# jiahuei/COMIC-Compact-Image-Captioning-with-Attention

Hardware: AMD Instinct MI355X
Metric: images/sec (decoder-mode XE training, COMIC-256, InceptionV3 frozen) (higher is better)
Workload: dtype bf16

## Files before the change

### comic-compact-image-captioning-with-attention_amd/_lib.py

```python
import ctypes as C
import os

_HERE = os.path.dirname(os.path.abspath(__file__))
LIB_PATH = os.environ.get('COMIC_HIP_LIB') or os.path.join(_HERE, 'lib', 'libcomic_hip.so')

c_void_p, c_int, c_int32, c_int64, c_float, c_double, c_char_p, c_uint64 = (
    C.c_void_p, C.c_int, C.c_int32, C.c_int64, C.c_float, C.c_double, C.c_char_p, C.c_uint64)


class CnnOp(C.Structure):
    _fields_ = [(n, c_int32) for n in (
        'kind', 'src', 'dst', 'src_coff', 'dst_coff', 'H', 'W', 'Cin', 'Cout', 'KH', 'KW', 'SH', 'SW',
        'PT', 'PL', 'Ho', 'Wo', 'weight', 'relu', 'out_f32', 'src_f32', 'lane', 'tile', 'group', 'flags', 'min_lds')]


class ImageDesc(C.Structure):
    _fields_ = [('offset', C.c_int64), ('in_h', c_int32), ('in_w', c_int32), ('flip', c_int32), ('oy', c_int32),
                ('ox', c_int32), ('sy', C.c_float), ('sx', C.c_float)]


class ConvWeight(C.Structure):
    _fields_ = [('w', c_void_p), ('scale', c_void_p), ('shift', c_void_p), ('w_frag', c_void_p)]


# ... 69 lines not shown


class BeamSampling(C.Structure):
    _fields_ = [('temperature', c_float), ('seed_dev', c_void_p)]


class BeamTruncation(C.Structure):
    _fields_ = [('top_k', c_int32), ('top_p', c_float)]


class GemmProb(C.Structure):
    _fields_ = [(n, c_void_p) for n in ('A', 'B', 'C', 'bias', 'mask')] + [(n, c_int32) for n in (
        'M', 'N', 'K', 'lda', 'ldb', 'ldc', 'ld_mask')] + [(n, c_float) for n in ('alpha', 'beta', 'keep')] + [
        ('type', c_int32), ('ones_a', c_int32)]


class ConvGrad(C.Structure):
    _fields_ = [('w_master', c_void_p), ('dw', c_void_p), ('dbeta', c_void_p), ('w_bwd', c_void_p),
                ('bwd_tile', c_int32), ('reserved', c_int32)]


P = c_void_p
_SIGS = {
    'comic_last_error': (c_char_p, []),
    'comic_abi_version': (c_int, []),
    'comic_device_count': (c_int, []),
    'comic_pack_conv_weights': (c_int, [P, P, c_int, c_int, c_int, c_int, c_int, P]),
    'comic_fold_bn': (c_int, [P, P, P, c_float, P, P, c_int, P]),
    'comic_cnn_forward': (c_int, [P, c_int, P, P, P, c_int, c_int, P]),
    'comic_cnn_group_args_bytes': (C.c_long, [P, c_int]),
    'comic_cnn_build_group_args': (c_int, [P, c_int, P, P, P, c_int, P]),
    'comic_cnn_forward_grouped': (c_int, [P, c_int, P, P, P, c_int, c_int, P, P]),
    'comic_clip_by_norm': (c_int, [P, P, P, c_int, c_float, c_float, c_float, P, P, P]),
    'comic_cnn_backward_scratch_bytes': (c_int64, [P, c_int, c_int, c_int, c_int]),
    'comic_cnn_backward': (c_int, [P, c_int, P, P, P, P, P, c_int, c_int, c_int, P, c_int64, P, P]),
    'comic_cnn_backward_sched': (c_int, [P, c_int, P, c_int, P, P, P, P, P, P, c_int, c_int, c_int, P, c_int64, P, P, P]),
    'comic_cnn_pack_bwd_filters': (c_int, [P, c_int, P, c_int, P]),
    'comic_cnn_pack_x3_weights': (c_int, [P, P, P, P, P, c_int, P]),
    'comic_cnn_refresh_weights': (c_int, [P, P, c_int64, P, P, P, P, c_int64, P]),
    'comic_cnn_refresh_weights_dtype': (c_int, [P, P, c_int64, P, P, P, P, c_int64, c_int, P]),
    'comic_cnn_pack_frag_weights': (c_int, [P, P, P, c_int, c_int64, P]),
    'comic_crc32c': (C.c_uint32, [P, C.c_size_t, C.c_uint32]),
    'comic_conv2d_bn_relu': (c_int, [P, P, c_int, P, c_int, P, c_int, c_int, P]),
    'comic_gemm_f32': (c_int, [P, P, P, P, c_int, c_int, c_int, c_int, c_int, c_int, c_int, c_int, c_float,
                               c_float, P]),
    'comic_gemm_f32_split3': (c_int, [P, P, P, P, c_int, c_int, c_int, c_int, c_int, c_int, c_int, c_int, c_float,
                                      c_float, P, c_int64, P]),
    'comic_gemm_f32_splitk': (c_int, [P, P, P, P, c_int, c_int, c_int, c_int, c_int, c_int, c_int, c_int, c_float,
                                      c_float, P, c_int64, P]),
    'comic_gemm_group_workspace': (c_int64, [P, c_int]),
    'comic_gemm_group': (c_int, [P, c_int, P, c_int64, P]),
    'comic_gemm_group_form': (c_int, [P, c_int, P, c_int64, c_int, P]),
    'comic_gemm_group_resident': (c_int, [c_int]),
    'comic_embed_fwd': (c_int, [P, P, P, c_int, c_int, c_int, P]),
    'comic_embed_bwd': (c_int, [P, P, P, c_int, c_int, c_int, P]),
    'comic_dropout_apply': (c_int, [P, P, c_float, P, c_int64, P]),
    'comic_dropout_mask': (c_int, [P, c_int64, c_float, c_uint64, c_uint64, P]),
    'comic_dropout_mask_dev': (c_int, [P, c_int64, c_float, P, c_uint64, P]),
    'comic_dropout_masks4_dev': (c_int, [P, P, P, P, P]),
    'comic_image_preprocess': (c_int, [P, P, c_int, P, c_int, c_int, c_int, P]),
    'comic_jpeg_pixels': (c_int, [P, P, c_int, c_int, c_int, c_int, P, P, P]),
    'comic_jpeg_preprocess': (c_int, [P, P, c_int, c_int, P, P, P, P, c_int, c_int, c_int, P]),
    'comic_jpeg_preprocess_packed': (c_int, [P, P, c_int, c_int, P, P, P, P, c_int, c_int, c_int, P]),
    'comic_weighted_sum_tb': (c_int, [P, P, c_int, c_int, P, P]),
    'comic_lstm_gates_fwd': (c_int, [P, P, P, P, P, P, P, P, c_float, P, c_int, P, P, c_int, c_int, P]),
    'comic_lstm_gates_bwd': (c_int, [P, P, P, P, P, c_float, P, c_int, P, P, P, c_int, c_int, P]),
    'comic_attn_step_fwd': (c_int, [P, P, P, P, P, P, P, P, P, c_float, P, P, P, P]),
    'comic_attn_step_bwd': (c_int, [P, P, P, P, P, P, P, P, P, P, c_float, P, P, P, P, P, P, P]),
    'comic_xent_fwd_bwd': (c_int, [P, P, P, P, P, P, P, P, c_int, c_int, c_int, P]),
    'comic_argmax_rows': (c_int, [P, P, c_int, c_int, P]),
    'comic_beam_step': (c_int, [P, P, P, P, P, P, P, c_int, c_int, c_int, c_int, P]),
    'comic_gather_rows': (c_int, [P, P, P, c_int, c_int, c_int, P]),
    'comic_gather_tree': (c_int, [P, P, P, P, c_int, c_int, c_int, c_int, P]),
    'comic_adam_tf': (c_int, [P, P, P, P, c_int64, c_float, c_float, c_float, c_float, c_float, c_float, P]),
    'comic_adam_tf_gated': (c_int, [P, P, P, P, c_int64, c_float, c_float, c_float, c_float, c_float, c_float, P, P]),
    'comic_momentum_tf_gated': (c_int, [P, P, P, c_int64, c_float, c_float, c_float, c_float, P, P]),
    'comic_debug_occupy_cus': (c_int, [c_int, c_int, P]),
    'comic_colsum': (c_int, [P, P, c_int, c_int, c_float, P]),
    'comic_ln_tanh_fwd': (c_int, [P, P, P, P, P, c_int, c_int, c_float, P]),
    'comic_ln_tanh_bwd_rows': (c_int, [P, P, P, P, P, c_int, c_int, P]),
    'comic_momentum_tf': (c_int, [P, P, P, c_int64, c_float, c_float, c_float, c_float, P]),
    'comic_axpy': (c_int, [P, P, c_float, c_int64, P]),
    'comic_decoder_train_workspace': (c_int64, [P, c_int, c_int]),
    'comic_decoder_train_path': (c_int, []),
    'comic_decoder_greedy_path': (c_int, []),
    'comic_decoder_beam_path': (c_int, []),
    'comic_beam_step_dense_workspace': (c_int64, [c_int, c_int, c_int, c_int]),
    'comic_beam_step_dense': (c_int, [c_void_p] * 9 + [c_int] * 5 + [c_void_p, c_int64, c_void_p]),
    'comic_gemm_f32_stream_workspace': (c_int64, [c_int, c_int, c_int]),
    'comic_gemm_f32_stream': (c_int, [c_void_p, c_void_p, c_void_p, c_void_p, c_int, c_int, c_int, c_void_p, c_int64, c_void_p]),
    'comic_decoder_infer_workspace': (c_int64, [P, c_int, c_int]),
    'comic_decoder_train_step': (c_int, [P, P, P, P, P, P, P, P, P, P, c_int, c_int, c_int, P, P, P, P, P, P, P,
                                         P, P, P, P, P, c_int64, P]),
    'comic_decoder_score_workspace': (c_int64, [P, c_int, c_int]),
    'comic_decoder_score': (c_int, [P, P, P, P, P, P, P, P, c_int, c_int, c_int, P, P, P, P, c_int64, P]),
    'comic_decoder_score_path': (c_int, []),
    'comic_decoder_greedy': (c_int, [P, P, P, P, c_int, c_int, P, P, P, P, P, c_int64, P]),
    'comic_decoder_sample': (c_int, [P, P, P, P, c_int, c_int, P, P, P, P, P, P, c_int64, P]),
    'comic_decoder_beam': (c_int, [P, P, P, P, c_int, c_int, c_int, P, P, P, P, P, P, P, P, c_int64, P]),
    'comic_beam_step_ensemble_workspace': (c_int64, [c_int, c_int, c_int, c_int]),
    'comic_beam_step_ensemble': (c_int, [P, P, c_int, P, P, P, P, P, P, c_int, c_int, c_int, c_int, c_float, P, c_int64, P]),
    'comic_beam_step_ensemble_path': (c_int, []),
    'comic_decoder_beam_ensemble_workspace': (c_int64, [P, c_int, c_int, c_int]),
    'comic_decoder_beam_ensemble': (c_int, [P, P, P, P, P, c_int, c_int, c_int, c_int, P, P, P, P, P, P, P, P, c_int64, P]),
    'comic_beam_bans': (c_int, [P, P, P, P, P, P, c_int, c_int, c_int, c_int, c_int, c_int, P, P]),
    'comic_beam_step_constrained': (c_int, [P, P, c_int, P, P, P, P, P, P, c_int, c_int, c_int, c_int, c_float, P, c_int, P,
# ... 166 lines not shown
```

### comic-compact-image-captioning-with-attention_amd/csrc/decoder_exec.hip

```cpp
#include <atomic>
#include <stdlib.h>

#include <algorithm>
#include <string.h>

#include "common.h"
#include "decoder_math.h"
#include "decoder_persist.h"
#include "exec_entries.h"
#include "gemm_group.h"
#include "lstm_prep.h"
#include "lstm_stream_dev.h"

int comic_gemm_f32_ws(const float* A, const float* B, float* C, const float* bias, int M, int N, int K, int lda,
                      int ldb, int ldc, int trans_a, int trans_b, float alpha, float beta, void* ws, int64_t ws_bytes,
                      hipStream_t st);
int comic_embed_bwd_set(const int32_t* ids, const float* dout, float* dtable, int rows, int E, int V, hipStream_t st);
int comic_gemm_bf16x3_impl(const float* A, const float* B, float* C, const float* bias, int M, int N, int K, int lda,
                           int ldb, int ldc, int trans_a, int trans_b, float alpha, float beta, void* ws,
                           int64_t ws_bytes, hipStream_t st);
bool comic_score_stream_supported(int D, int V);
int64_t comic_score_logits_ws_bytes(int D, int V, long rows, int stream);
float* comic_score_logits_buffer(void* ws);
int comic_score_logits(const float* y, const float* W_o, const float* b_o, const int32_t* targets_bt, const float* wmask_bt,
// ... 407 lines not shown
  finished[i] = first ? 0 : 1;
  lengths[i] = 0;
}

__global__ void pad_rows_kernel(const float* __restrict__ in, float* __restrict__ out, int cols, int ld, long n) {
  const long i = (long)blockIdx.x * blockDim.x + threadIdx.x;
  if (i >= n) return;
  const long r = i / ld;
  const int c = (int)(i - r * ld);
  out[i] = c < cols ? in[r * cols + c] : 0.f;
}

inline int fill(float* p, float v, long n, hipStream_t st) {
  if (n <= 0) return 0;
  hipLaunchKernelGGL(fill_kernel, dim3((unsigned)cdiv64(n, 256)), dim3(256), 0, st, p, v, n);
  COMIC_LAUNCH_CHECK("fill");
  return 0;
}
constexpr int64_t kSplitKBytes = 32ll << 20;

inline int gemm(const float* A, const float* B, float* C, const float* bias, int M, int N, int K, int lda, int ldb,
                int ldc, int ta, int tb, float beta, hipStream_t st) {
  return comic_gemm_f32_ws(A, B, C, bias, M, N, K, lda, ldb, ldc, ta, tb, 1.0f, beta, g_splitk_ws,
                           g_splitk_ws ? kSplitKBytes : 0, st);
}

inline int gemm_big(const float* A, const float* B, float* C, const float* bias, int M, int N, int K, int lda, int ldb,
                    int ldc, int ta, int tb, float beta, hipStream_t st) {
  const bool on = !(g_dec_flags & COMIC_DEC_EXACT_GEMM);
  if (!on || (long)M * N < 64 * 256 || K < 64)
    return gemm(A, B, C, bias, M, N, K, lda, ldb, ldc, ta, tb, beta, st);
  return comic_gemm_bf16x3_impl(A, B, C, bias, M, N, K, lda, ldb, ldc, ta, tb, 1.0f, beta, g_splitk_ws,
                                g_splitk_ws ? kSplitKBytes : 0, st);
}

constexpr int kGroupTickets = 4096;
struct GemmGroupRun {
  ComicGemmGroup g{};
  ComicGemmProb* add(int type, const float* A, const float* B, float* C, int M, int N, int K, int lda, int ldb, int ldc) {
    if (g.n >= kGemmGroupMax) return nullptr;
    ComicGemmProb& p = g.p[g.n++];
    p = ComicGemmProb{};
    p.type = type; p.A = A; p.B = B; p.C = C; p.M = M; p.N = N; p.K = K; p.lda = lda; p.ldb = ldb; p.ldc = ldc;
    p.alpha = 1.f; p.beta = 0.f; p.keep = 1.f;
    return &p;
  }
  ComicGemmProb* add_colsum(const float* B, float* C, int N, int K, int ldb) {
    ComicGemmProb* p = add(COMIC_GG_TN, nullptr, B, C, 1, N, K, 1, ldb, N);
    if (p) p->ones_a = 1;
    return p;
  }
  int run(void* slab, int64_t slab_cap, unsigned* tickets, hipStream_t st) {
    if (g.n == 0) return 0;
    int target = kGemmGroupTargetItems;
    for (;;) {
      int64_t need = 0;
      int nt = 0;
      const int wg = comic_gemm_group_plan(g, target, &need, &nt);
      if (wg < 0) return 2;
      if (need <= slab_cap && nt <= kGroupTickets - 8) {
        g.slab = (float*)slab;
        g.tickets = tickets;
        return comic_gemm_group_launch(g, wg, st);
      }
      COMIC_REQUIRE(target > 1, "gemm_group: split-K scratch too small");
      target = target / 2;
    }
  }
};

int check_desc(const comic_decoder_desc* d) {
  COMIC_REQUIRE(d, "decoder: null descriptor");
  COMIC_REQUIRE(d->D > 0 && d->E > 0 && d->A > 0 && d->V > 1 && d->C > 0 && d->Cg > 0 && d->H > 0 && d->M > 0,
                "decoder: bad dimensions");
  const int cv = d->fm_projection == 0 ? d->C : d->D;
  COMIC_REQUIRE(d->Cv == cv, "decoder: Cv must be %d for fm_projection %d", cv, d->fm_projection);
  const int a = (d->fm_projection == 0 && !d->context_layer) ? d->C : d->D;
  COMIC_REQUIRE(d->A == a, "decoder: attention size A must be %d", a);
  COMIC_REQUIRE(d->cell >= COMIC_CELL_LSTM && d->cell <= COMIC_CELL_GRU, "decoder: unknown cell %d", d->cell);
  return 0;
}
int check_cell_params(const comic_decoder_desc* d, const comic_decoder_params* p) {
  COMIC_REQUIRE(p && p->K, "decoder: null cell kernel");
  if (d->cell == COMIC_CELL_LSTM) COMIC_REQUIRE(p->b, "decoder: LSTM needs its bias");
  if (d->cell == COMIC_CELL_LN_LSTM) COMIC_REQUIRE(p->cell_ln, "decoder: LN_LSTM needs cell_ln");
  if (d->cell == COMIC_CELL_GRU) COMIC_REQUIRE(p->b && p->K_c && p->b_c, "decoder: GRU needs b, K_c, b_c");
  return 0;
}

comic_attn_desc attn_desc(const comic_decoder_desc* d, int rows) {
  comic_attn_desc a;
  a.B = rows; a.M = d->M; a.D = d->D; a.H = d->H; a.Cv = d->Cv;
  a.method = d->method; a.prob = d->prob; a.tied = d->fm_projection == 2;
  return a;
}

int memory_projections(const comic_decoder_desc* d, const comic_decoder_params* p, const float* fm, int rows,
                       float* keys, float* values_buf, const float** values, hipStream_t st) {
  RC(gemm_big(fm, p->W_m, keys, nullptr, rows * d->M, d->D, d->C, d->C, d->D, d->D, 0, 0, 0.f, st));
  if (d->fm_projection == 2) {
    *values = keys;
  } else if (d->fm_projection == 1) {
    RC(gemm_big(fm, p->W_v, values_buf, nullptr, rows * d->M, d->D, d->C, d->C, d->D, d->D, 0, 0, 0.f, st));
    *values = values_buf;
  } else {
    *values = fm;
  }
  return 0;
}

struct InitBufs {
  float *x, *xh, *g, *gates, *c_new;
  float *lnx = nullptr, *lnr = nullptr;
};

int rnn_init_fwd(const comic_decoder_desc* d, const comic_decoder_params* p, const float* im_embed, int rows,
                 const float* mask_init, InitBufs& ib, float* c0, float* h0, hipStream_t st) {
  const int D = d->D, EA = d->E + d->A;
  if (d->init_method == 1) {
    RC(gemm(im_embed, p->W_init, h0, nullptr, rows, D, d->Cg, d->Cg, D, D, 0, 0, 0.f, st));
// ... 1655 lines not shown
```

### comic-compact-image-captioning-with-attention_amd/csrc/gemm_group.h

```cpp
#pragma once
#include "common.h"

constexpr int kGemmGroupMax = 20;
enum { COMIC_GG_TN = 0, COMIC_GG_NN = 1, COMIC_GG_NT = 2 };

struct ComicGemmProb {
  const float* A;
  const float* B;
  float* C;
  const float* bias;
  const float* mask;
  int M, N, K, lda, ldb, ldc, ld_mask;
  float alpha, beta;
  float keep;
  int type;
  int ones_a;
  int tiles_m, tiles_n, S, k_per_slice, wg_begin;
  int slab_tile0;
  int ticket0;
};

struct ComicGemmGroup {
  ComicGemmProb p[kGemmGroupMax];
  int n;
  float* slab;
  unsigned* tickets;
  int xcd_chunk;
};

int comic_gemm_group_plan(ComicGemmGroup& g, int target_items, int64_t* slab_bytes, int* n_tickets);
constexpr int kGemmGroupTargetItems = 640;
int comic_gemm_group_launch(const ComicGemmGroup& g, int n_wg, hipStream_t st, int form = 0);
```

### comic-compact-image-captioning-with-attention_amd/csrc/gemm_group.hip

```cpp
#include <algorithm>

#include "gemm_group.h"
#include "gemm_x3_dev.h"

namespace {

constexpr int GB = 128;
constexpr int kGemmGroupSlots = 512;
constexpr int kItemOverhead = 6;
constexpr int kSc1 = 16;
typedef __attribute__((ext_vector_type(4))) unsigned gg_u32x4_t;

__device__ __forceinline__ __amdgpu_buffer_rsrc_t gg_rsrc(const void* p, long bytes) {
  return __builtin_amdgcn_make_buffer_rsrc((void*)p, 0, (int)bytes, 0x00020000);
}
__device__ __forceinline__ float4 gg_load16_sc1(__amdgpu_buffer_rsrc_t r, unsigned off) {
  const gg_u32x4_t v = __builtin_amdgcn_raw_buffer_load_b128(r, (int)off, 0, kSc1);
  return make_float4(__uint_as_float(v.x), __uint_as_float(v.y), __uint_as_float(v.z), __uint_as_float(v.w));
}
__device__ __forceinline__ void gg_store16_sc1(__amdgpu_buffer_rsrc_t r, unsigned off, float4 v) {
  const gg_u32x4_t u = {__float_as_uint(v.x), __float_as_uint(v.y), __float_as_uint(v.z), __float_as_uint(v.w)};
  __builtin_amdgcn_raw_buffer_store_b128(u, r, (int)off, 0, kSc1);
}

constexpr int kGroupLds = 4 * (X3Tile<GB, true>::BYTES + X3Tile<GB, true>::BYTES);
static_assert(X3Tile<GB, true>::BYTES >= X3Tile<GB, false>::BYTES, "LDS of the k-contiguous form bounds the others");
constexpr int kGroupLdsPc = 2 * 2 * (X3TilePc<GB, false>::BYTES + X3TilePc<GB, false>::BYTES);
static_assert(X3TilePc<GB, false>::BYTES >= X3TilePc<GB, true>::BYTES, "LDS of the row-contiguous form bounds the others");

__device__ __forceinline__ void gg_emit(const ComicGemmProb& p, int m, int n, float4 a) {
  if (m >= p.M || n >= p.N) return;
  const int nv = min(4, p.N - n);
  float v[4] = {a.x * p.alpha, a.y * p.alpha, a.z * p.alpha, a.w * p.alpha};
  float* cp = p.C + (size_t)m * p.ldc + n;
#pragma unroll
  for (int q = 0; q < 4; ++q) {
    if (q >= nv) break;
    if (p.bias) v[q] += p.bias[n + q];
    if (p.mask) v[q] = (v[q] / p.keep) * p.mask[(size_t)m * p.ld_mask + n + q];
    if (p.beta != 0.f) v[q] += p.beta * cp[q];
  }
  if (nv == 4 && (p.ldc % 4 == 0) && (((uintptr_t)p.C & 15) == 0)) {
    *(float4*)cp = make_float4(v[0], v[1], v[2], v[3]);
  } else {
#pragma unroll
    for (int q = 0; q < 4; ++q)
      if (q < nv) cp[q] = v[q];
  }
}

template <int FORM>
__global__ __launch_bounds__(FORM == 1 ? 256 : 512)
#if defined(__HIP_DEVICE_COMPILE__)
__attribute__((amdgpu_waves_per_eu(FORM == 3 ? 4 : 1, FORM == 3 ? 4 : 2)))
#endif
void gemm_group_x3_kernel(ComicGemmGroup g) {
  constexpr bool PC = FORM != 1;
  constexpr int NT = PC ? 512 : 256;
  constexpr int LDS = PC ? kGroupLdsPc : kGroupLds;
  extern __shared__ __attribute__((aligned(16))) unsigned char smem[];
  int bid = blockIdx.x;
  if (g.xcd_chunk > 0 && bid < g.xcd_chunk * 8) bid = (bid & 7) * g.xcd_chunk + (bid >> 3);
  volatile unsigned* s_last = (volatile unsigned*)(smem + LDS - 16);
  int pi = 0;
#pragma unroll 1
  for (int i = 1; i < g.n; ++i)
    if (bid >= g.p[i].wg_begin) pi = i;
  const ComicGemmProb& p = g.p[pi];
  const int local = bid - p.wg_begin;
  const int S = p.S, ntiles = p.tiles_m * p.tiles_n;
  const int slice = local / ntiles, tl = local - slice * ntiles;
  constexpr int PW = 8;
  const int panel = tl / (p.tiles_m * PW), rem = tl - panel * p.tiles_m * PW;
  const int pw = min(PW, p.tiles_n - panel * PW);
  const int mt = rem / pw, nt = panel * PW + rem % pw;
  const int tile = mt * p.tiles_n + nt;
  const int m0 = mt * GB, n0 = nt * GB;
  const int kbeg = S > 1 ? slice * p.k_per_slice : 0;
  const int kend = S > 1 ? min(p.K, kbeg + p.k_per_slice) : p.K;
  const int tid = threadIdx.x, lane = tid & 63, wave = tid >> 6;
  const int wm = wave >> 1, wn = wave & 1;

  const long tile_id = (long)p.ticket0 + tile;
  const __amdgpu_buffer_rsrc_t sr = gg_rsrc(g.slab + ((long)p.slab_tile0 + (long)tile * S) * (GB * GB), (long)S * GB * GB * 4);
  const unsigned sbase = (unsigned)slice * (GB * GB * 4);
  if (p.ones_a) {
    constexpr int KG = 8;
    float4* red = (float4*)smem;
    const int cg = tid & 31, kg = tid >> 5, n = n0 + 4 * cg;
    const bool vec = (p.ldb % 4 == 0) && (((uintptr_t)p.B & 15) == 0);
    float4 sm = make_float4(0.f, 0.f, 0.f, 0.f);
    if (n < p.N && kg < KG)
      for (int k = kbeg + kg; k < kend; k += KG) {
        const float4 v = load4(p.B + (size_t)k * p.ldb + n, p.N - n, vec);
        sm.x += v.x; sm.y += v.y; sm.z += v.z; sm.w += v.w;
      }
    if (kg < KG) red[kg * 32 + cg] = sm;
    __syncthreads();
    if (tid < 32) {
      float4 tot = red[cg];
#pragma unroll
      for (int k = 1; k < KG; ++k) {
        const float4 v = red[k * 32 + cg];
        tot.x += v.x; tot.y += v.y; tot.z += v.z; tot.w += v.w;
      }
      if (S == 1) gg_emit(p, 0, n, tot);
      else gg_store16_sc1(sr, sbase + (unsigned)cg * 16u, tot);
    }
    if (S == 1) return;
  } else {
    f32x4_t acc[4][4];
    if constexpr (PC) {
      constexpr int DEPTH = FORM == 3 ? 2 : 4;
      if (p.type == COMIC_GG_TN) x3_mainloop_pc<false, false, DEPTH>(p.A, p.B, p.M, p.N, p.lda, p.ldb, m0, n0, kbeg, kend, smem, acc);
      else if (p.type == COMIC_GG_NN) x3_mainloop_pc<true, false, DEPTH>(p.A, p.B, p.M, p.N, p.lda, p.ldb, m0, n0, kbeg, kend, smem, acc);
      else x3_mainloop_pc<true, true, DEPTH>(p.A, p.B, p.M, p.N, p.lda, p.ldb, m0, n0, kbeg, kend, smem, acc);
    } else {
      if (p.type == COMIC_GG_TN)
        x3_mainloop<GB, false, false, GB>(p.A, p.B, p.M, p.N, p.lda, p.ldb, m0, n0, kbeg, kend, smem, acc);
      else if (p.type == COMIC_GG_NN)
        x3_mainloop<GB, true, false, GB>(p.A, p.B, p.M, p.N, p.lda, p.ldb, m0, n0, kbeg, kend, smem, acc);
      else
        x3_mainloop<GB, true, true, GB>(p.A, p.B, p.M, p.N, p.lda, p.ldb, m0, n0, kbeg, kend, smem, acc);
    }
    const bool owner = wave < 4;
    if (S == 1) {
      if (owner)
#pragma unroll
      for (int i = 0; i < 4; ++i)
#pragma unroll
        for (int j = 0; j < 4; ++j)
          gg_emit(p, m0 + wm * 64 + j * 16 + (lane & 15), n0 + wn * 64 + i * 16 + (lane >> 4) * 4,
                  make_float4(acc[i][j][0], acc[i][j][1], acc[i][j][2], acc[i][j][3]));
      return;
    }
    if (owner)
#pragma unroll
    for (int i = 0; i < 4; ++i)
#pragma unroll
      for (int j = 0; j < 4; ++j) {
        const int ml = wm * 64 + j * 16 + (lane & 15), nl = wn * 64 + i * 16 + (lane >> 4) * 4;
        gg_store16_sc1(sr, sbase + (unsigned)(ml * GB + nl) * 4u, make_float4(acc[i][j][0], acc[i][j][1], acc[i][j][2], acc[i][j][3]));
      }
  }
  asm volatile("s_waitcnt vmcnt(0)" ::: "memory");
  __syncthreads();
  if (tid == 0) {
    const unsigned t = __hip_atomic_fetch_add(g.tickets + tile_id, 1u, __ATOMIC_RELAXED, __HIP_MEMORY_SCOPE_AGENT);
    *s_last = (t == (unsigned)(S - 1)) ? 1u : 0u;
    if (t == (unsigned)(S - 1)) __hip_atomic_store(g.tickets + tile_id, 0u, __ATOMIC_RELAXED, __HIP_MEMORY_SCOPE_AGENT);
  }
  __syncthreads();
  if (!*s_last) return;
  const int n_chunks = p.ones_a ? 1 : (GB * GB / 4) / NT;
#pragma unroll 1
  for (int c = 0; c < n_chunks; c += 4) {
    float4 sum[4];
#pragma unroll
    for (int u = 0; u < 4; ++u) sum[u] = make_float4(0.f, 0.f, 0.f, 0.f);
#pragma unroll 1
    for (int s = 0; s < S; ++s) {
      float4 v[4];
#pragma unroll
      for (int u = 0; u < 4; ++u) v[u] = gg_load16_sc1(sr, (unsigned)s * (GB * GB * 4) + (unsigned)(tid + NT * (c + u)) * 16u);
#pragma unroll
      for (int u = 0; u < 4; ++u) {
        sum[u].x += v[u].x; sum[u].y += v[u].y; sum[u].z += v[u].z; sum[u].w += v[u].w;
      }
    }
#pragma unroll
    for (int u = 0; u < 4; ++u) {
      const int idx4 = tid + NT * (c + u);
      if (!p.ones_a || idx4 < GB / 4) gg_emit(p, m0 + idx4 / (GB / 4), n0 + (idx4 % (GB / 4)) * 4, sum[u]);
    }
  }
}


}

int comic_gemm_group_plan(ComicGemmGroup& g, int target_items, int64_t* slab_bytes, int* n_tickets) {
  COMIC_REQUIRE(g.n > 0 && g.n <= kGemmGroupMax, "gemm_group: %d problems", g.n);
  long cost = 0;
  for (int i = 0; i < g.n; ++i) {
    ComicGemmProb& p = g.p[i];
    COMIC_REQUIRE(p.M > 0 && p.N > 0 && p.K > 0 && p.B && p.C && (p.A || p.ones_a), "gemm_group: bad problem %d", i);
    COMIC_REQUIRE(p.type >= COMIC_GG_TN && p.type <= COMIC_GG_NT, "gemm_group: bad type of problem %d", i);
    COMIC_REQUIRE(!p.ones_a || (p.type == COMIC_GG_TN && p.M == 1), "gemm_group: ones_a needs type TN and M = 1 (problem %d)", i);
    COMIC_REQUIRE(p.ldc >= p.N && (!p.mask || p.ld_mask >= p.N), "gemm_group: leading dimension of problem %d", i);
    if (!p.ones_a) COMIC_REQUIRE(p.lda >= (p.type == COMIC_GG_TN ? p.M : p.K), "gemm_group: lda of problem %d", i);
    COMIC_REQUIRE(p.ldb >= (p.type == COMIC_GG_NT ? p.K : p.N), "gemm_group: ldb of problem %d", i);
    p.tiles_m = cdiv(p.M, GB);
    p.tiles_n = cdiv(p.N, GB);
    cost += (long)cdiv(p.M, GB) * p.tiles_n * cdiv(p.K, 32);
  }
  auto split_of = [](int kt, long klen) { return (int)std::min<long>(16, std::max<long>(1, (kt + klen / 2) / klen)); };
  long klen = std::max<long>(8, cost / std::max(1, target_items));
  {
    long best = -1, best_klen = klen, kt_max = 8;
    for (int i = 0; i < g.n; ++i) kt_max = std::max<long>(kt_max, cdiv(g.p[i].K, 32));
    for (long kl = klen; kl <= kt_max; ++kl) {
      long items = 0, longest = 0;
      for (int i = 0; i < g.n; ++i) {
        const ComicGemmProb& p = g.p[i];
        const int kt = cdiv(p.K, 32), S = split_of(kt, kl);
        items += (long)p.tiles_m * p.tiles_n * S;
        if (!p.ones_a) longest = std::max<long>(longest, cdiv(kt, S));
      }
      const long est = cdiv64(items, kGemmGroupSlots) * (longest + kItemOverhead);
      if (best < 0 || est < best) {
        best = est;
        best_klen = kl;
      }
    }
    klen = best_klen;
  }
  int wg = 0, tickets = 0, slab_tiles = 0;
  for (int i = 0; i < g.n; ++i) {
    ComicGemmProb& p = g.p[i];
    const int nt = cdiv(p.M, GB) * p.tiles_n, kt = cdiv(p.K, 32);
    int S = split_of(kt, klen);
    p.k_per_slice = cdiv(kt, S) * 32;
    S = cdiv(p.K, p.k_per_slice);
    p.S = S;
    p.wg_begin = wg;
    p.slab_tile0 = slab_tiles;
    p.ticket0 = tickets;
    wg += nt * S;
    if (S > 1) {
      slab_tiles += nt * S;
      tickets += nt;
    }
  }
  if (slab_bytes) *slab_bytes = (int64_t)slab_tiles * GB * GB * 4;
  if (n_tickets) *n_tickets = tickets;
  return wg;
}

namespace {
bool gg_vec_ok(const ComicGemmGroup& g) {
  for (int i = 0; i < g.n; ++i) {
    const ComicGemmProb& p = g.p[i];
    if (p.ones_a) continue;
    const bool a_kc = p.type != COMIC_GG_TN, b_kc = p.type == COMIC_GG_NT;
    if (!(p.lda % 4 == 0 && p.ldb % 4 == 0 && ((uintptr_t)p.A & 15) == 0 && ((uintptr_t)p.B & 15) == 0 &&
          (!(a_kc || b_kc) || p.K % 4 == 0)))
      return false;
  }
  return true;
}
const void* gg_kernel(int form) {
  return form == 1 ? (const void*)gemm_group_x3_kernel<1> : form == 2 ? (const void*)gemm_group_x3_kernel<2> : (const void*)gemm_group_x3_kernel<3>;
}
int gg_lds(int form) { return form == 1 ? kGroupLds : kGroupLdsPc; }
int gg_reserve_lds(int form) {
  static PerDeviceOnce once[3];
  bool& done = once[form - 1].slot();
  if (!done) {
    COMIC_REQUIRE(hipFuncSetAttribute(gg_kernel(form), hipFuncAttributeMaxDynamicSharedMemorySize, gg_lds(form)) == hipSuccess,
                  "gemm_group: cannot reserve %d bytes of LDS", gg_lds(form));
    done = true;
  }
  return 0;
}
}

int comic_gemm_group_launch(const ComicGemmGroup& g_in, int n_wg, hipStream_t st, int form) {
  ComicGemmGroup g = g_in;
  g.xcd_chunk = n_wg / 8;
  COMIC_REQUIRE(n_wg > 0, "gemm_group: empty launch");
  COMIC_REQUIRE(form >= 0 && form <= 3, "gemm_group: form %d", form);
  const bool vec = gg_vec_ok(g);
  if (form == 0) form = vec ? 3 : 1;
  COMIC_REQUIRE(form == 1 || vec, "gemm_group: form %d needs 16-byte loadable operands", form);
  if (int rc = gg_reserve_lds(form)) return rc;
  if (form == 1) hipLaunchKernelGGL(gemm_group_x3_kernel<1>, dim3((unsigned)n_wg), dim3(256), kGroupLds, st, g);
  else if (form == 2) hipLaunchKernelGGL(gemm_group_x3_kernel<2>, dim3((unsigned)n_wg), dim3(512), kGroupLdsPc, st, g);
  else hipLaunchKernelGGL(gemm_group_x3_kernel<3>, dim3((unsigned)n_wg), dim3(512), kGroupLdsPc, st, g);
  COMIC_LAUNCH_CHECK("gemm_group");
  return 0;
}

namespace {
int gg_from_public(const comic_gemm_prob* probs, int n, ComicGemmGroup& g) {
  COMIC_REQUIRE(probs && n > 0 && n <= kGemmGroupMax, "gemm_group: 1..%d problems", kGemmGroupMax);
  g = ComicGemmGroup{};
  g.n = n;
  for (int i = 0; i < n; ++i) {
    const comic_gemm_prob& q = probs[i];
    ComicGemmProb& p = g.p[i];
    p.A = q.A; p.B = q.B; p.C = q.C; p.bias = q.bias; p.mask = q.mask;
    p.M = q.M; p.N = q.N; p.K = q.K; p.lda = q.lda; p.ldb = q.ldb; p.ldc = q.ldc; p.ld_mask = q.ld_mask;
    p.alpha = q.alpha; p.beta = q.beta; p.keep = q.keep; p.type = q.type; p.ones_a = q.ones_a;
  }
  return 0;
}
#define kPublicTarget kGemmGroupTargetItems
}

extern "C" int64_t comic_gemm_group_workspace(const comic_gemm_prob* probs, int n) {
  ComicGemmGroup g;
  if (gg_from_public(probs, n, g)) return -1;
  int64_t slab = 0;
  int nt = 0;
  if (comic_gemm_group_plan(g, kPublicTarget, &slab, &nt) < 0) return -1;
  return slab + 256 + (int64_t)nt * 4;
}

extern "C" int comic_gemm_group_form(const comic_gemm_prob* probs, int n, void* workspace, int64_t workspace_bytes, int form,
                                     void* stream) {
  COMIC_REQUIRE(form >= 0 && form <= 3, "gemm_group: form %d", form);
  ComicGemmGroup g;
  if (int rc = gg_from_public(probs, n, g)) return rc;
  int64_t slab = 0;
  int nt = 0;
  const int wg = comic_gemm_group_plan(g, kPublicTarget, &slab, &nt);
  if (wg < 0) return 2;
  COMIC_REQUIRE(form < 2 || gg_vec_ok(g), "gemm_group: form %d needs 16-byte loadable operands", form);
  const int64_t slab_al = (slab + 255) / 256 * 256;
  COMIC_REQUIRE(nt == 0 || (workspace && workspace_bytes >= slab_al + (int64_t)nt * 4), "gemm_group: workspace too small");
  g.slab = (float*)workspace;
  g.tickets = nt ? (unsigned*)((char*)workspace + slab_al) : nullptr;
  if (nt) COMIC_REQUIRE(hipMemsetAsync(g.tickets, 0, (size_t)nt * 4, (hipStream_t)stream) == hipSuccess, "gemm_group: memset");
  return comic_gemm_group_launch(g, wg, (hipStream_t)stream, form);
}

extern "C" int comic_gemm_group(const comic_gemm_prob* probs, int n, void* workspace, int64_t workspace_bytes, void* stream) {
  return comic_gemm_group_form(probs, n, workspace, workspace_bytes, 0, stream);
}

extern "C" int comic_gemm_group_resident(int form) {
  if (form < 1 || form > 3) {
    comic_set_error("gemm_group: form %d", form);
    return -1;
  }
  if (gg_reserve_lds(form)) return -1;
  int nb = 0;
  if (hipOccupancyMaxActiveBlocksPerMultiprocessor(&nb, gg_kernel(form), form == 1 ? 256 : 512, gg_lds(form)) != hipSuccess) {
    comic_set_error("gemm_group: occupancy query failed");
    return -1;
  }
  return nb;
}
```

### include/comic_hip.h

```cpp
#ifndef COMIC_HIP_H_
#define COMIC_HIP_H_

#include <stddef.h>
#include <stdint.h>

#ifdef __cplusplus
extern "C" {
#endif

#define COMIC_F32 0
#define COMIC_BF16 1
#define COMIC_F16 2
#define COMIC_ABI_VERSION 1
#define COMIC_CONV_TILES 61
#define COMIC_WS_TILE 54
#define COMIC_IMG_TILE 55
#define COMIC_CHAIN_TILE 62

const char* comic_last_error(void);
int comic_abi_version(void);
int comic_device_count(void);


int comic_pack_conv_weights(const float* w_hwio, void* w_packed, int kh, int kw, int cin, int cout,
// ... 72 lines not shown
  int32_t reserved;
} comic_conv_grad;
int64_t comic_cnn_backward_scratch_bytes(const comic_cnn_op* ops, int n_ops, int batch, int dtype, int lanes);
int comic_cnn_backward(const comic_cnn_op* ops, int n_ops, void* const* buffers,
                       void* const* grad_buffers, const int32_t* buf_channels,
                       const comic_conv_weight* weights, const comic_conv_grad* grads, int batch,
                       int dtype, int filters_ready ,
                       void* scratch, int64_t scratch_bytes, void* stream, void* wgrad_stream);
#define COMIC_CNN_BWD_NO_ACT_FUSION 2
int comic_cnn_backward_sched(const comic_cnn_op* ops, int n_ops, const int32_t* sched, int n_sched, void* const* buffers,
                             void* const* grad_buffers, void* const* grad_buffers_alt, const int32_t* buf_channels,
                             const comic_conv_weight* weights, const comic_conv_grad* grads, int batch, int dtype,
                             int filters_ready, void* scratch, int64_t scratch_bytes, void* stream0, void* stream1,
                             void* wgrad_stream);
int comic_cnn_pack_x3_weights(const float* const* masters, void* const* outs, const int32_t* cout, const int32_t* taps,
                              const int32_t* cin, int n, void* stream);
int comic_cnn_pack_bwd_filters(const comic_cnn_op* ops, int n_ops, const comic_conv_grad* grads,
                               int dtype, void* stream);
int comic_cnn_refresh_weights(const float* master, void* plan_copy, int64_t n, const float* beta,
                              const float* mean, const float* scale, float* shift,
                              int64_t channels, void* stream);
int comic_cnn_refresh_weights_dtype(const float* master, void* plan_copy, int64_t n, const float* beta,
                                    const float* mean, const float* scale, float* shift,
                                    int64_t channels, int dtype, void* stream);

int comic_conv2d_bn_relu(const comic_cnn_op* op, const void* x, int x_channels, void* y,
                         int y_channels, const comic_conv_weight* wt, int batch, int dtype,
                         void* stream);

int comic_gemm_f32(const float* A, const float* B, float* C, const float* bias, int M, int N, int K,
                   int lda, int ldb, int ldc, int trans_a, int trans_b, float alpha, float beta,
                   void* stream);

int comic_gemm_f32_split3(const float* A, const float* B, float* C, const float* bias, int M, int N,
                          int K, int lda, int ldb, int ldc, int trans_a, int trans_b, float alpha,
                          float beta, void* workspace ,
                          int64_t workspace_bytes, void* stream);

typedef struct comic_gemm_prob {
  const float* A;
  const float* B;
  float* C;
  const float* bias;
  const float* mask;
  int32_t M, N, K, lda, ldb, ldc, ld_mask;
  float alpha, beta, keep;
  int32_t type, ones_a;
} comic_gemm_prob;
int64_t comic_gemm_group_workspace(const comic_gemm_prob* probs, int n);
int comic_gemm_group(const comic_gemm_prob* probs, int n, void* workspace, int64_t workspace_bytes, void* stream);
int comic_gemm_group_form(const comic_gemm_prob* probs, int n, void* workspace, int64_t workspace_bytes, int form,
                          void* stream);
int comic_gemm_group_resident(int form);

int64_t comic_gemm_f32_stream_workspace(int R, int Kin, int N);
int comic_gemm_f32_stream(const float* x, const float* W, const float* bias, float* out, int R, int Kin, int N,
                          void* workspace, int64_t workspace_bytes, void* stream);

int comic_gemm_f32_splitk(const float* A, const float* B, float* C, const float* bias, int M, int N,
                          int K, int lda, int ldb, int ldc, int trans_a, int trans_b, float alpha,
                          float beta, void* workspace, int64_t workspace_bytes, void* stream);

int comic_embed_fwd(const float* table, const int32_t* ids, float* out, int rows, int E, int V,
                    void* stream);
int comic_embed_bwd(const int32_t* ids, const float* dout, float* dtable, int rows, int E, int V,
                    void* stream);

int comic_dropout_apply(const float* x, const float* mask, float keep, float* y, int64_t n,
                        void* stream);
int comic_dropout_mask(float* mask, int64_t n, float keep, uint64_t seed, uint64_t offset,
                       void* stream);
int comic_dropout_mask_dev(float* mask, int64_t n, float keep, const uint64_t* seed_dev,
                           uint64_t offset, void* stream);
int comic_dropout_masks4_dev(float* mask, const int64_t* n4, const float* keep4, const uint64_t* seed_dev,
                             void* stream);
int comic_weighted_sum_tb(const float* rows_tb, const float* w_bt, int T, int B, float* out, void* stream);

int comic_lstm_gates_fwd(const float* g, const float* c_prev, const float* h_prev, float* gates_act,
                         float* c_new, float* h_new, float* y, const float* mask_out, float keep_out,
                         const int32_t* lens, int t, float* c_state, float* h_state, int B, int D,
                         void* stream);
int comic_lstm_gates_bwd(const float* gates_act, const float* c_prev, const float* c_new,
                         const float* dy, const float* mask_out, float keep_out, const int32_t* lens,
                         int t, float* dc_state, float* dh_state, float* dg, int B, int D, void* stream);

typedef struct comic_attn_desc {
  int32_t B, M, D, H, Cv;
  int32_t method;
  int32_t prob;
  int32_t tied;
} comic_attn_desc;

int comic_attn_step_fwd(const comic_attn_desc* d, const float* keys, const float* values,
                        const float* q, const float* ln_g, const float* ln_b, const float* v,
                        const float* tau, const float* mask_alpha, float keep_alpha, float* alpha,
                        float* alpha_d, float* ctx, void* stream);
int comic_attn_step_bwd(const comic_attn_desc* d, const float* keys, const float* values,
                        const float* q, const float* ln_g, const float* ln_b, const float* v,
                        const float* tau, const float* alpha, const float* mask_alpha,
                        float keep_alpha, const float* dctx, const float* dmap, float* dq,
                        float* dkeys, float* dvalues, float* pgrad, void* stream);

int comic_xent_fwd_bwd(float* logits, const int32_t* targets_bt, const float* coef_bt,
                       const float* wmask_bt, const int32_t* lens, float* loss_rows, float* dlogits,
                       int32_t* ids_tb, int T, int B, int V, void* stream);

// ... 308 lines not shown
```

Baseline: 40280.

## Add 64x64 tile path to grouped GEMM with cost-model split-K planning

Adds a 64-edge tile variant to the grouped split-K GEMM kernel. The planner picks it for problems with M<=64 or for small launches, and picks its K-split length from a cost model of items per slot and combine overhead. The aim is better occupancy of the 512 workgroup slots when small decoder GEMMs would otherwise leave most CUs idle with 128x128 tiles. It also adds public entry points for forced tile and split choices, plus plan introspection. Risks: smaller tiles mean less data reuse per tile, and the hand-tuned cost constants may pick poor splits.

```diff
diff --git a/comic-compact-image-captioning-with-attention_amd/_lib.py b/comic-compact-image-captioning-with-attention_amd/_lib.py
--- a/comic-compact-image-captioning-with-attention_amd/_lib.py
+++ b/comic-compact-image-captioning-with-attention_amd/_lib.py
@@ -145,6 +145,8 @@
     'comic_gemm_group': (c_int, [P, c_int, P, c_int64, P]),
     'comic_gemm_group_form': (c_int, [P, c_int, P, c_int64, c_int, P]),
     'comic_gemm_group_resident': (c_int, [c_int]),
+    'comic_gemm_group_tiles': (c_int, [P, c_int, P, c_int64, c_int, c_int, c_int, P]),
+    'comic_gemm_group_plan_info': (c_int, [P, c_int, c_int, c_int, c_int, P, P, P]),
     'comic_embed_fwd': (c_int, [P, P, P, c_int, c_int, c_int, P]),
     'comic_embed_bwd': (c_int, [P, P, P, c_int, c_int, c_int, P]),
     'comic_dropout_apply': (c_int, [P, P, c_float, P, c_int64, P]),
diff --git a/comic-compact-image-captioning-with-attention_amd/csrc/decoder_exec.hip b/comic-compact-image-captioning-with-attention_amd/csrc/decoder_exec.hip
--- a/comic-compact-image-captioning-with-attention_amd/csrc/decoder_exec.hip
+++ b/comic-compact-image-captioning-with-attention_amd/csrc/decoder_exec.hip
@@ -483,20 +483,7 @@
   }
   int run(void* slab, int64_t slab_cap, unsigned* tickets, hipStream_t st) {
     if (g.n == 0) return 0;
-    int target = kGemmGroupTargetItems;
-    for (;;) {
-      int64_t need = 0;
-      int nt = 0;
-      const int wg = comic_gemm_group_plan(g, target, &need, &nt);
-      if (wg < 0) return 2;
-      if (need <= slab_cap && nt <= kGroupTickets - 8) {
-        g.slab = (float*)slab;
-        g.tickets = tickets;
-        return comic_gemm_group_launch(g, wg, st);
-      }
-      COMIC_REQUIRE(target > 1, "gemm_group: split-K scratch too small");
-      target = target / 2;
-    }
+    return comic_gemm_group_run(g, slab, slab_cap, tickets, kGroupTickets - 8, st);
   }
 };
 
diff --git a/comic-compact-image-captioning-with-attention_amd/csrc/gemm_group.h b/comic-compact-image-captioning-with-attention_amd/csrc/gemm_group.h
--- a/comic-compact-image-captioning-with-attention_amd/csrc/gemm_group.h
+++ b/comic-compact-image-captioning-with-attention_amd/csrc/gemm_group.h
@@ -16,7 +16,8 @@
   int type;
   int ones_a;
   int tiles_m, tiles_n, S, k_per_slice, wg_begin;
-  int slab_tile0;
+  int tb;
+  int slab_off;
   int ticket0;
 };
 
@@ -28,6 +29,9 @@
   int xcd_chunk;
 };
 
-int comic_gemm_group_plan(ComicGemmGroup& g, int target_items, int64_t* slab_bytes, int* n_tickets);
+int comic_gemm_group_plan(ComicGemmGroup& g, int target_items, int64_t* slab_bytes, int* n_tickets, int force_tb = 0,
+                          int force_S = 0);
 constexpr int kGemmGroupTargetItems = 640;
+int comic_gemm_group_run(ComicGemmGroup& g, void* slab, int64_t slab_cap, unsigned* tickets, int ticket_cap, hipStream_t st,
+                         int form = 0, int force_tb = 0, int force_S = 0);
 int comic_gemm_group_launch(const ComicGemmGroup& g, int n_wg, hipStream_t st, int form = 0);
diff --git a/comic-compact-image-captioning-with-attention_amd/csrc/gemm_group.hip b/comic-compact-image-captioning-with-attention_amd/csrc/gemm_group.hip
--- a/comic-compact-image-captioning-with-attention_amd/csrc/gemm_group.hip
+++ b/comic-compact-image-captioning-with-attention_amd/csrc/gemm_group.hip
@@ -6,8 +6,11 @@
 namespace {
 
 constexpr int GB = 128;
+constexpr int GS = 64;
 constexpr int kGemmGroupSlots = 512;
 constexpr int kItemOverhead = 6;
+constexpr double kOverhead64 = 1.6, kKtile64 = 0.38, kCombineFix64 = 3.5, kCombine64 = 0.7;
+constexpr int kMinLen64 = 2;
 constexpr int kSc1 = 16;
 typedef __attribute__((ext_vector_type(4))) unsigned gg_u32x4_t;
 
@@ -46,6 +49,34 @@
 #pragma unroll
     for (int q = 0; q < 4; ++q)
       if (q < nv) cp[q] = v[q];
+  }
+}
+
+template <int TBX, int NTHR>
+__device__ __forceinline__ void gg_combine(const ComicGemmProb& p, __amdgpu_buffer_rsrc_t sr, int S, int m0, int n0, int tid) {
+  constexpr int ROW4 = TBX / 4;
+  static_assert((TBX * TBX / 4) % (4 * NTHR) == 0, "four float4 per thread and round");
+  const int n_chunks = p.ones_a ? 1 : (TBX * TBX / 4) / NTHR;
+#pragma unroll 1
+  for (int c = 0; c < n_chunks; c += 4) {
+    float4 sum[4];
+#pragma unroll
+    for (int u = 0; u < 4; ++u) sum[u] = make_float4(0.f, 0.f, 0.f, 0.f);
+#pragma unroll 1
+    for (int s = 0; s < S; ++s) {
+      float4 v[4];
+#pragma unroll
+      for (int u = 0; u < 4; ++u) v[u] = gg_load16_sc1(sr, (unsigned)s * (TBX * TBX * 4) + (unsigned)(tid + NTHR * (c + u)) * 16u);
+#pragma unroll
+      for (int u = 0; u < 4; ++u) {
+        sum[u].x += v[u].x; sum[u].y += v[u].y; sum[u].z += v[u].z; sum[u].w += v[u].w;
+      }
+    }
+#pragma unroll
+    for (int u = 0; u < 4; ++u) {
+      const int idx4 = tid + NTHR * (c + u);
+      if (!p.ones_a || idx4 < ROW4) gg_emit(p, m0 + idx4 / ROW4, n0 + (idx4 % ROW4) * 4, sum[u]);
+    }
   }
 }
 
@@ -75,15 +106,18 @@
   const int pw = min(PW, p.tiles_n - panel * PW);
   const int mt = rem / pw, nt = panel * PW + rem % pw;
   const int tile = mt * p.tiles_n + nt;
-  const int m0 = mt * GB, n0 = nt * GB;
+  const int TB = p.tb;
+  const int m0 = mt * TB, n0 = nt * TB;
   const int kbeg = S > 1 ? slice * p.k_per_slice : 0;
   const int kend = S > 1 ? min(p.K, kbeg + p.k_per_slice) : p.K;
-  const int tid = threadIdx.x, lane = tid & 63, wave = tid >> 6;
+  const int tid = threadIdx.x, lane = tid & 63;
+  const int wave = __builtin_amdgcn_readfirstlane(tid >> 6);
   const int wm = wave >> 1, wn = wave & 1;
 
   const long tile_id = (long)p.ticket0 + tile;
-  const __amdgpu_buffer_rsrc_t sr = gg_rsrc(g.slab + ((long)p.slab_tile0 + (long)tile * S) * (GB * GB), (long)S * GB * GB * 4);
-  const unsigned sbase = (unsigned)slice * (GB * GB * 4);
+  const long tile_floats = (long)TB * TB;
+  const __amdgpu_buffer_rsrc_t sr = gg_rsrc(g.slab + (long)p.slab_off + (long)tile * S * tile_floats, (long)S * tile_floats * 4);
+  const unsigned sbase = (unsigned)slice * (unsigned)(tile_floats * 4);
   if (p.ones_a) {
     constexpr int KG = 8;
     float4* red = (float4*)smem;
@@ -107,6 +141,29 @@
       if (S == 1) gg_emit(p, 0, n, tot);
       else gg_store16_sc1(sr, sbase + (unsigned)cg * 16u, tot);
     }
+    if (S == 1) return;
+  } else if (TB == GS) {
+    if constexpr (PC)
+      if (wave >= 4) return;
+    f32x4_t acc[2][2];
+    if constexpr (PC) {
+      if (p.type == COMIC_GG_TN) x3_mainloop_v<GS, false, false, GS, true>(p.A, p.B, p.M, p.N, p.lda, p.ldb, m0, n0, kbeg, kend, smem, acc);
+      else if (p.type == COMIC_GG_NN) x3_mainloop_v<GS, true, false, GS, true>(p.A, p.B, p.M, p.N, p.lda, p.ldb, m0, n0, kbeg, kend, smem, acc);
+      else x3_mainloop_v<GS, true, true, GS, true>(p.A, p.B, p.M, p.N, p.lda, p.ldb, m0, n0, kbeg, kend, smem, acc);
+    } else {
+      if (p.type == COMIC_GG_TN) x3_mainloop<GS, false, false, GS>(p.A, p.B, p.M, p.N, p.lda, p.ldb, m0, n0, kbeg, kend, smem, acc);
+      else if (p.type == COMIC_GG_NN) x3_mainloop<GS, true, false, GS>(p.A, p.B, p.M, p.N, p.lda, p.ldb, m0, n0, kbeg, kend, smem, acc);
+      else x3_mainloop<GS, true, true, GS>(p.A, p.B, p.M, p.N, p.lda, p.ldb, m0, n0, kbeg, kend, smem, acc);
+    }
+#pragma unroll
+    for (int i = 0; i < 2; ++i)
+#pragma unroll
+      for (int j = 0; j < 2; ++j) {
+        const int ml = wm * 32 + j * 16 + (lane & 15), nl = wn * 32 + i * 16 + (lane >> 4) * 4;
+        const float4 v = make_float4(acc[i][j][0], acc[i][j][1], acc[i][j][2], acc[i][j][3]);
+        if (S == 1) gg_emit(p, m0 + ml, n0 + nl, v);
+        else gg_store16_sc1(sr, sbase + (unsigned)(ml * GS + nl) * 4u, v);
+      }
     if (S == 1) return;
   } else {
     f32x4_t acc[4][4];
@@ -152,35 +209,16 @@
   }
   __syncthreads();
   if (!*s_last) return;
-  const int n_chunks = p.ones_a ? 1 : (GB * GB / 4) / NT;
-#pragma unroll 1
-  for (int c = 0; c < n_chunks; c += 4) {
-    float4 sum[4];
-#pragma unroll
-    for (int u = 0; u < 4; ++u) sum[u] = make_float4(0.f, 0.f, 0.f, 0.f);
-#pragma unroll 1
-    for (int s = 0; s < S; ++s) {
-      float4 v[4];
-#pragma unroll
-      for (int u = 0; u < 4; ++u) v[u] = gg_load16_sc1(sr, (unsigned)s * (GB * GB * 4) + (unsigned)(tid + NT * (c + u)) * 16u);
-#pragma unroll
-      for (int u = 0; u < 4; ++u) {
-        sum[u].x += v[u].x; sum[u].y += v[u].y; sum[u].z += v[u].z; sum[u].w += v[u].w;
-      }
-    }
-#pragma unroll
-    for (int u = 0; u < 4; ++u) {
-      const int idx4 = tid + NT * (c + u);
-      if (!p.ones_a || idx4 < GB / 4) gg_emit(p, m0 + idx4 / (GB / 4), n0 + (idx4 % (GB / 4)) * 4, sum[u]);
-    }
-  }
-}
-
-
-}
-
-int comic_gemm_group_plan(ComicGemmGroup& g, int target_items, int64_t* slab_bytes, int* n_tickets) {
+  if (TB == GS) gg_combine<GS, 256>(p, sr, S, m0, n0, tid);
+  else gg_combine<GB, NT>(p, sr, S, m0, n0, tid);
+}
+
+}
+
+int comic_gemm_group_plan(ComicGemmGroup& g, int target_items, int64_t* slab_bytes, int* n_tickets, int force_tb, int force_S) {
   COMIC_REQUIRE(g.n > 0 && g.n <= kGemmGroupMax, "gemm_group: %d problems", g.n);
+  COMIC_REQUIRE(force_tb == 0 || force_tb == GS || force_tb == GB, "gemm_group: tile edge %d", force_tb);
+  COMIC_REQUIRE(force_S >= 0 && force_S <= 16, "gemm_group: split %d", force_S);
   long cost = 0;
   for (int i = 0; i < g.n; ++i) {
     ComicGemmProb& p = g.p[i];
@@ -190,6 +228,7 @@
     COMIC_REQUIRE(p.ldc >= p.N && (!p.mask || p.ld_mask >= p.N), "gemm_group: leading dimension of problem %d", i);
     if (!p.ones_a) COMIC_REQUIRE(p.lda >= (p.type == COMIC_GG_TN ? p.M : p.K), "gemm_group: lda of problem %d", i);
     COMIC_REQUIRE(p.ldb >= (p.type == COMIC_GG_NT ? p.K : p.N), "gemm_group: ldb of problem %d", i);
+    p.tb = GB;
     p.tiles_m = cdiv(p.M, GB);
     p.tiles_n = cdiv(p.N, GB);
     cost += (long)cdiv(p.M, GB) * p.tiles_n * cdiv(p.K, 32);
@@ -215,24 +254,78 @@
     }
     klen = best_klen;
   }
-  int wg = 0, tickets = 0, slab_tiles = 0;
+  long items128 = 0;
   for (int i = 0; i < g.n; ++i) {
     ComicGemmProb& p = g.p[i];
-    const int nt = cdiv(p.M, GB) * p.tiles_n, kt = cdiv(p.K, 32);
+    const int kt = cdiv(p.K, 32);
     int S = split_of(kt, klen);
+    if (force_S && !p.ones_a) S = std::min(force_S, kt);
     p.k_per_slice = cdiv(kt, S) * 32;
-    S = cdiv(p.K, p.k_per_slice);
-    p.S = S;
+    p.S = cdiv(p.K, p.k_per_slice);
+    items128 += (long)p.tiles_m * p.tiles_n * p.S;
+  }
+  const bool small_launch = items128 < kGemmGroupSlots / 2;
+  long fixed_items = 0, n64 = 0;
+  double long128 = 0.0;
+  for (int i = 0; i < g.n; ++i) {
+    ComicGemmProb& p = g.p[i];
+    const bool e64 = !p.ones_a && (force_tb ? force_tb == GS : (p.M <= GS || small_launch));
+    if (e64) {
+      p.tb = GS;
+      p.tiles_m = cdiv(p.M, GS);
+      p.tiles_n = cdiv(p.N, GS);
+      ++n64;
+    } else {
+      fixed_items += (long)p.tiles_m * p.tiles_n * p.S;
+      if (!p.ones_a) long128 = std::max(long128, (double)(cdiv(p.K, p.S * 32) + kItemOverhead));
+    }
+  }
+  if (n64 && !force_S) {
+    const long min_len = target_items >= kGemmGroupTargetItems ? kMinLen64 : std::max<long>(kMinLen64, cost / std::max(1, target_items));
+    long kt_max = min_len;
+    for (int i = 0; i < g.n; ++i)
+      if (g.p[i].tb == GS) kt_max = std::max<long>(kt_max, cdiv(g.p[i].K, 32));
+    double best = -1.0;
+    long best_kl = kt_max;
+    for (long kl = kt_max; kl >= min_len; --kl) {
+      long items = fixed_items;
+      double longest64 = 0.0;
+      for (int i = 0; i < g.n; ++i) {
+        const ComicGemmProb& p = g.p[i];
+        if (p.tb != GS) continue;
+        const int kt = cdiv(p.K, 32), S = split_of(kt, kl), len = cdiv(kt, S), Se = cdiv(kt, len);
+        items += (long)p.tiles_m * p.tiles_n * Se;
+        longest64 = std::max(longest64, kOverhead64 + kKtile64 * len + (Se > 1 ? kCombineFix64 + kCombine64 * Se : 0.0));
+      }
+      const double est = (double)cdiv64(items, kGemmGroupSlots) * std::max(long128, longest64);
+      if (best < 0 || est < best) {
+        best = est;
+        best_kl = kl;
+      }
+    }
+    for (int i = 0; i < g.n; ++i) {
+      ComicGemmProb& p = g.p[i];
+      if (p.tb != GS) continue;
+      const int kt = cdiv(p.K, 32);
+      p.k_per_slice = cdiv(kt, split_of(kt, best_kl)) * 32;
+      p.S = cdiv(p.K, p.k_per_slice);
+    }
+  }
+  int wg = 0, tickets = 0;
+  int64_t slab_floats = 0;
+  for (int i = 0; i < g.n; ++i) {
+    ComicGemmProb& p = g.p[i];
+    const int nt = p.tiles_m * p.tiles_n;
     p.wg_begin = wg;
-    p.slab_tile0 = slab_tiles;
+    p.slab_off = (int)std::min<int64_t>(slab_floats, 0x7FFFFFFF);
     p.ticket0 = tickets;
-    wg += nt * S;
-    if (S > 1) {
-      slab_tiles += nt * S;
+    wg += nt * p.S;
+    if (p.S > 1) {
+      slab_floats += (int64_t)nt * p.S * p.tb * p.tb;
       tickets += nt;
     }
   }
-  if (slab_bytes) *slab_bytes = (int64_t)slab_tiles * GB * GB * 4;
+  if (slab_bytes) *slab_bytes = slab_floats * 4;
   if (n_tickets) *n_tickets = tickets;
   return wg;
 }
@@ -281,6 +374,24 @@
   return 0;
 }
 
+int comic_gemm_group_run(ComicGemmGroup& g, void* slab, int64_t slab_cap, unsigned* tickets, int ticket_cap, hipStream_t st,
+                         int form, int force_tb, int force_S) {
+  int target = kGemmGroupTargetItems;
+  for (;;) {
+    int64_t need = 0;
+    int nt = 0;
+    const int wg = comic_gemm_group_plan(g, target, &need, &nt, force_tb, force_S);
+    if (wg < 0) return 2;
+    if (need <= slab_cap && nt <= ticket_cap && need < (8ll << 30)) {
+      g.slab = (float*)slab;
+      g.tickets = tickets;
+      return comic_gemm_group_launch(g, wg, st, form);
+    }
+    COMIC_REQUIRE(target > 1 && !force_S, "gemm_group: split-K scratch too small");
+    target = target / 2;
+  }
+}
+
 namespace {
 int gg_from_public(const comic_gemm_prob* probs, int n, ComicGemmGroup& g) {
   COMIC_REQUIRE(probs && n > 0 && n <= kGemmGroupMax, "gemm_group: 1..%d problems", kGemmGroupMax);
@@ -317,6 +428,7 @@
   const int wg = comic_gemm_group_plan(g, kPublicTarget, &slab, &nt);
   if (wg < 0) return 2;
   COMIC_REQUIRE(form < 2 || gg_vec_ok(g), "gemm_group: form %d needs 16-byte loadable operands", form);
+  COMIC_REQUIRE(slab < (8ll << 30), "gemm_group: split-K scratch of 8 GiB or more");
   const int64_t slab_al = (slab + 255) / 256 * 256;
   COMIC_REQUIRE(nt == 0 || (workspace && workspace_bytes >= slab_al + (int64_t)nt * 4), "gemm_group: workspace too small");
   g.slab = (float*)workspace;
@@ -329,6 +441,36 @@
   return comic_gemm_group_form(probs, n, workspace, workspace_bytes, 0, stream);
 }
 
+constexpr int kPublicTickets = 4096;
+extern "C" int comic_gemm_group_tiles(const comic_gemm_prob* probs, int n, void* workspace, int64_t workspace_bytes, int form,
+                                      int tile_edge, int split, void* stream) {
+  COMIC_REQUIRE(form >= 0 && form <= 3, "gemm_group: form %d", form);
+  ComicGemmGroup g;
+  if (int rc = gg_from_public(probs, n, g)) return rc;
+  COMIC_REQUIRE(form < 2 || gg_vec_ok(g), "gemm_group: form %d needs 16-byte loadable operands", form);
+  const int64_t head = (int64_t)kPublicTickets * 4;
+  COMIC_REQUIRE(workspace && workspace_bytes >= head, "gemm_group: workspace too small");
+  return comic_gemm_group_run(g, (char*)workspace + head, workspace_bytes - head, (unsigned*)workspace, kPublicTickets,
+                              (hipStream_t)stream, form, tile_edge, split);
+}
+
+extern "C" int comic_gemm_group_plan_info(const comic_gemm_prob* probs, int n, int target_items, int tile_edge, int split,
+                                          int32_t* info, int64_t* slab_bytes, int32_t* n_tickets) {
+  ComicGemmGroup g;
+  if (gg_from_public(probs, n, g)) return -1;
+  int nt = 0;
+  const int wg = comic_gemm_group_plan(g, target_items > 0 ? target_items : kGemmGroupTargetItems, slab_bytes, &nt, tile_edge, split);
+  if (wg < 0) return -1;
+  if (n_tickets) *n_tickets = nt;
+  if (info)
+    for (int i = 0; i < n; ++i) {
+      const ComicGemmProb& p = g.p[i];
+      const int32_t v[6] = {p.tb, p.tiles_m, p.tiles_n, p.S, p.k_per_slice, p.wg_begin};
+      for (int j = 0; j < 6; ++j) info[i * 6 + j] = v[j];
+    }
+  return wg;
+}
+
 extern "C" int comic_gemm_group_resident(int form) {
   if (form < 1 || form > 3) {
     comic_set_error("gemm_group: form %d", form);
diff --git a/include/comic_hip.h b/include/comic_hip.h
--- a/include/comic_hip.h
+++ b/include/comic_hip.h
@@ -148,6 +148,10 @@
 int comic_gemm_group_form(const comic_gemm_prob* probs, int n, void* workspace, int64_t workspace_bytes, int form,
                           void* stream);
 int comic_gemm_group_resident(int form);
+int comic_gemm_group_tiles(const comic_gemm_prob* probs, int n, void* workspace, int64_t workspace_bytes, int form,
+                           int tile_edge, int split, void* stream);
+int comic_gemm_group_plan_info(const comic_gemm_prob* probs, int n, int target_items, int tile_edge, int split, int32_t* info,
+                               int64_t* slab_bytes, int32_t* n_tickets);
 
 int64_t comic_gemm_f32_stream_workspace(int R, int Kin, int N);
 int comic_gemm_f32_stream(const float* x, const float* W, const float* bias, float* out, int R, int Kin, int N,
```

New measurement: 40460, median of 6. No clear change (+0.4%).
